# Stansfash/nonstationary-precip

Hardware: NVIDIA B200
Metric: SVGP-Gibbs ELBO steps/s (higher is better)
Workload: dtype f64

## Files before the change

nonstationary_precip_b200/csrc/common.cuh:

```cuda
#pragma once
#include <cuda_runtime.h>
#include <stdint.h>

#define NPGP_OK 0
#define NPGP_EINVAL (-1)
#define NPGP_EUNSUPPORTED (-2)
#define NPGP_EWORKSPACE (-3)

extern "C" long npgp_launch_counter;

#define NPGP_LAUNCH_CHECK()                       \
  do {                                            \
    ++npgp_launch_counter;                        \
    cudaError_t e__ = cudaGetLastError();         \
    if (e__ != cudaSuccess) return (int)e__;      \
  } while (0)

#define NPGP_CUDA(call)                           \
  do {                                            \
    cudaError_t e__ = (call);                     \
    if (e__ != cudaSuccess) return (int)e__;      \
  } while (0)

namespace npgp {

constexpr int kNumSMs = 148;

__device__ __forceinline__ double warp_sum(double v) {
#pragma unroll
  for (int o = 16; o > 0; o >>= 1) v += __shfl_xor_sync(0xffffffffu, v, o);
  return v;
}

__device__ __forceinline__ double block_sum(double v, double* smem ) {
  const int lane = threadIdx.x & 31, w = threadIdx.x >> 5;
  v = warp_sum(v);
  if (lane == 0) smem[w] = v;
  __syncthreads();
  double r = 0.0;
  if (w == 0) {
    r = (lane < (int)((blockDim.x + 31) >> 5)) ? smem[lane] : 0.0;
    r = warp_sum(r);
  }
  __syncthreads();
  return r;
}

__device__ __forceinline__ void st_v2(double* p, double a, double b) {
  *reinterpret_cast<double2*>(p) = make_double2(a, b);
}

static inline int ceil_div(long a, long b) { return (int)((a + b - 1) / b); }

template <int NRC>
struct RowReducer {
  static constexpr int RB = (32 / NRC) > 0 ? (32 / NRC) : 1;
  static constexpr int LINES = RB * NRC;
  static constexpr int PANEL = LINES * 33;
  double* panel;
  int lane;
  __device__ __forceinline__ RowReducer(double* smem_base, int warp, int lane_) : panel(smem_base + warp * PANEL), lane(lane_) {}
  __device__ __forceinline__ void put(int r, int comp, double v) { panel[((r % RB) * NRC + comp) * 33 + lane]  = v; }
  template <class F>
  __device__ __forceinline__ void flush_if_due(int r, int nr, F out) {
    const int slot = r % RB;
    if (slot != RB - 1 && r != nr - 1) return;
    __syncwarp();
    const int nvals = (slot + 1) * NRC;
    for (int v = lane; v < nvals; v += 32) {
      const double* line = panel + v * 33;
      double a0 = 0.0, a1 = 0.0, a2 = 0.0, a3 = 0.0;
#pragma unroll
      for (int k = 0; k < 32; k += 4) {
        a0 += line[k];
        a1 += line[k + 1];
        a2 += line[k + 2];
        a3 += line[k + 3];
      }
      out(r - slot + v / NRC, v % NRC, (a0 + a1) + (a2 + a3));
    }
    __syncwarp();
  }
};

constexpr int kNT = 128;
constexpr int kCPT = 2;
constexpr int kTJ = kNT * kCPT;
constexpr int kTI = 32;

struct GSpec {
  const double* Gm;
  long ldg;
  const double* rowscale;
  const double* rowvec;
  const double* colvec;
};

#ifndef NPGP_GPF_DEPTH
#define NPGP_GPF_DEPTH 4
#endif
template <int CPT, int DEPTH = NPGP_GPF_DEPTH>
struct GPrefetch {
  const double* base;
  long ldg;
  int row_end;
  bool v[CPT], vec;
  double q[DEPTH][CPT];
  __device__ __forceinline__ GPrefetch(const GSpec& g, int jbase, const bool* valid, int vec_ok, int row_begin,
                                       int row_end_)
      : base(g.Gm ? g.Gm + jbase : nullptr), ldg(g.ldg), row_end(row_end_) {
#pragma unroll
    for (int c = 0; c < CPT; ++c) v[c] = valid[c];
    vec = (CPT == 2) && vec_ok && valid[CPT - 1];
#pragma unroll
    for (int k = 0; k < DEPTH; ++k) fetch(row_begin + k, q[k]);
  }
  __device__ __forceinline__ void fetch(int i, double* out) const {
#pragma unroll
    for (int c = 0; c < CPT; ++c) out[c] = 0.0;
    if (base == nullptr || i >= row_end) return;
    const double* grow = base + (long)i * ldg;
    if (vec) {
      const double2 t = *reinterpret_cast<const double2*>(grow);
      out[0] = t.x;
      out[CPT - 1] = t.y;
    } else {
#pragma unroll
      for (int c = 0; c < CPT; ++c)
        if (v[c]) out[c] = grow[c];
    }
  }
  __device__ __forceinline__ void pop(int i, double* out) {
#pragma unroll
    for (int c = 0; c < CPT; ++c) out[c] = q[0][c];
#pragma unroll
    for (int k = 0; k + 1 < DEPTH; ++k)
#pragma unroll
      for (int c = 0; c < CPT; ++c) q[k][c] = q[k + 1][c];
    fetch(i + DEPTH, q[DEPTH - 1]);
  }
};

static inline int pick_rows_per_cta(int n1, int col_tiles, int waves_target) {
  long want = (long)kNumSMs * waves_target;
  long row_ctas = (want + col_tiles - 1) / col_tiles;
  long rpc = (n1 + row_ctas - 1) / row_ctas;
  rpc = ((rpc + kTI - 1) / kTI) * kTI;
  if (rpc < kTI) rpc = kTI;
  return (int)rpc;
}

}
```

nonstationary_precip_b200/csrc/gibbs_full.cu:

```cuda
#include <cstdlib>
#include "common.cuh"
#include "pairmath.cuh"

namespace npgp {


template <int d>
__device__ __forceinline__ void stage_rows_full(int n1, int i0, const double* __restrict__ x1,
                                                const double* __restrict__ S1, double (*sx)[d],
                                                double (*sS)[sym_size(d)], double* sq) {
  constexpr int P = sym_size(d);
  for (int r = threadIdx.x; r < kTI; r += kNT) {
    const int i = i0 + r;
    double S[P];
#pragma unroll
    for (int k = 0; k < d; ++k) sx[r][k] = (i < n1) ? x1[(long)i * d + k] : 0.0;
#pragma unroll
    for (int p = 0; p < P; ++p) S[p] = 0.0;
#pragma unroll
    for (int k = 0; k < d; ++k) S[sym_idx(d, k, k)] = 1.0;
    if (i < n1) {
#pragma unroll
      for (int p = 0; p < P; ++p) S[p] = S1[(long)i * P + p];
    }
#pragma unroll
    for (int p = 0; p < P; ++p) sS[r][p] = S[p];
    sq[r] = sqrt(sqrt(sym_det<d>(S)));
  }
}

template <int d>
__device__ __forceinline__ void load_col_full(int n2, int j, const double* __restrict__ x2,
                                              const double* __restrict__ S2, double* z, double* S, double& q,
                                              bool& valid) {
  constexpr int P = sym_size(d);
  valid = j < n2;
#pragma unroll
  for (int k = 0; k < d; ++k) z[k] = valid ? x2[(long)j * d + k] : 0.0;
#pragma unroll
  for (int p = 0; p < P; ++p) S[p] = 0.0;
#pragma unroll
  for (int k = 0; k < d; ++k) S[sym_idx(d, k, k)] = 1.0;
  if (valid) {
#pragma unroll
    for (int p = 0; p < P; ++p) S[p] = S2[(long)j * P + p];
  }
  q = full_col_factor<d>(sym_det<d>(S));
}

template <int d, bool HAS_U>
__global__ void __launch_bounds__(kNT) gibbs_full_fwd_kernel(int n1, int n2, const double* __restrict__ x1,
                                                             const double* __restrict__ S1,
                                                             const double* __restrict__ x2,
                                                             const double* __restrict__ S2, double jit2,
                                                             const double* __restrict__ scale, double* __restrict__ K,
                                                             long ldk, int vec_ok, const double* __restrict__ u,
                                                             double* __restrict__ Ku, int rows_per_cta) {
  constexpr int P = sym_size(d);
  __shared__ double sx[kTI][d], sS[kTI][P], sq[kTI];
  __shared__ double sexp[256];
  load_exp_table(sexp);
  const int jbase = blockIdx.y * kTJ + threadIdx.x * kCPT;
  const int row_begin = blockIdx.x * rows_per_cta;
  const int row_end = min(n1, row_begin + rows_per_cta);
  const double s = scale ? *scale : 1.0;
  double z[kCPT][d], Sj[kCPT][P], qj[kCPT], uj[kCPT];
  bool valid[kCPT];
#pragma unroll
  for (int c = 0; c < kCPT; ++c) {
    load_col_full<d>(n2, jbase + c, x2, S2, z[c], Sj[c], qj[c], valid[c]);
    qj[c] *= s;
    uj[c] = (HAS_U && valid[c]) ? u[jbase + c] : 0.0;
  }
  for (int i0 = row_begin; i0 < row_end; i0 += kTI) {
    __syncthreads();
    stage_rows_full<d>(n1, i0, x1, S1, sx, sS, sq);
    __syncthreads();
    const int nr = min(kTI, row_end - i0);
#pragma unroll 2
    for (int r = 0; r < nr; ++r) {
      const double k0 = gibbs_full_eval<d>(sx[r], sS[r], sq[r], z[0], Sj[0], qj[0], jit2, sexp);
      const double k1 = gibbs_full_eval<d>(sx[r], sS[r], sq[r], z[1], Sj[1], qj[1], jit2, sexp);
      double* krow = K + (long)(i0 + r) * ldk + jbase;
      if (vec_ok && valid[1]) {
        st_v2(krow, k0, k1);
      } else {
        if (valid[0]) krow[0] = k0;
        if (valid[1]) krow[1] = k1;
      }
      if (HAS_U) {
        double p = warp_sum(fma(k0, uj[0], k1 * uj[1]));
        if ((threadIdx.x & 31) == 0) atomicAdd(&Ku[i0 + r], p);
      }
    }
  }
}


#ifndef NPGP_FULL_BWD_MINB
#define NPGP_FULL_BWD_MINB 2
#endif
template <int d, bool DX1, bool DX2, int CPT>
__global__ void __launch_bounds__(kNT, NPGP_FULL_BWD_MINB) gibbs_full_bwd_kernel(int n1, int n2, const double* __restrict__ x1,
                                                             const double* __restrict__ S1,
                                                             const double* __restrict__ x2,
                                                             const double* __restrict__ S2, double jit2,
                                                             const double* __restrict__ scale, GSpec g, int vec_ok,
                                                             double* __restrict__ d_S1, double* __restrict__ d_x1,
                                                             double* __restrict__ d_S2, double* __restrict__ d_x2,
                                                             double* __restrict__ d_scale, int rows_per_cta) {
  constexpr int P = sym_size(d);
  constexpr int NRC = P + 1 + (DX1 ? d : 0);
  constexpr int NW = kNT / 32;
  __shared__ double sx[kTI][d], sS[kTI][P], sq[kTI], srs[kTI], srv[kTI];
  __shared__ double part[NW][kTI][NRC];
  __shared__ double red[32];
  __shared__ double panels[NW * RowReducer<NRC>::PANEL];
  const int lane = threadIdx.x & 31, warp = threadIdx.x >> 5;
  RowReducer<NRC> rr(panels, warp, lane);
  __shared__ double sexp[256];
  load_exp_table(sexp);
  const int jbase = blockIdx.y * (kNT * CPT) + threadIdx.x * CPT;
  const int row_begin = blockIdx.x * rows_per_cta;
  const int row_end = min(n1, row_begin + rows_per_cta);
  const double s = scale ? *scale : 1.0;
  double z[CPT][d], Sj[CPT][P], qj[CPT], cv[CPT];
  bool valid[CPT];
#pragma unroll
  for (int c = 0; c < CPT; ++c) {
    load_col_full<d>(n2, jbase + c, x2, S2, z[c], Sj[c], qj[c], valid[c]);
    cv[c] = (g.colvec && valid[c]) ? g.colvec[jbase + c] : 0.0;
    qj[c] *= s;
  }
  double cW[CPT][P], cs0[CPT], cxz[CPT][d];
#pragma unroll
  for (int c = 0; c < CPT; ++c) {
    cs0[c] = 0.0;
#pragma unroll
    for (int p = 0; p < P; ++p) cW[c][p] = 0.0;
#pragma unroll
    for (int k = 0; k < d; ++k) cxz[c][k] = 0.0;
  }
  GPrefetch<CPT> gq(g, jbase, valid, vec_ok, row_begin, row_end);

  for (int i0 = row_begin; i0 < row_end; i0 += kTI) {
    __syncthreads();
    stage_rows_full<d>(n1, i0, x1, S1, sx, sS, sq);
    for (int r = threadIdx.x; r < kTI; r += kNT) {
      const int i = i0 + r;
      srs[r] = (g.rowscale && i < n1) ? g.rowscale[i] : 1.0;
      srv[r] = (g.rowvec && i < n1) ? g.rowvec[i] : 0.0;
    }
    __syncthreads();
    const int nr = min(kTI, row_end - i0);
    for (int r = 0; r < nr; ++r) {
      double gv[CPT];
      gq.pop(i0 + r, gv);
#pragma unroll
      for (int c = 0; c < CPT; ++c) gv[c] = fma(srv[r], cv[c], gv[c] * srs[r]);
      double rW[P], rxz[d], rs0 = 0.0;
#pragma unroll
      for (int p = 0; p < P; ++p) rW[p] = 0.0;
#pragma unroll
      for (int k = 0; k < d; ++k) rxz[k] = 0.0;
#pragma unroll
      for (int c = 0; c < CPT; ++c) {
        FullPair<d> pr;
        gibbs_full_eval<d>(sx[r], sS[r], sq[r], z[c], Sj[c], qj[c], jit2, sexp, &pr);
        const double gk = valid[c] ? gv[c] * pr.k : 0.0;
        rs0 += gk;
        cs0[c] += gk;
        const double c2 = -gk * pr.hr2;
        double t[d];
#pragma unroll
        for (int a = 0; a < d; ++a) t[a] = (0.5 * gk) * pr.w[a];
#pragma unroll
        for (int a = 0; a < d; ++a)
#pragma unroll
          for (int b = a; b < d; ++b) {
            const int p = sym_idx(d, a, b);
            const double w = fma(t[a], pr.w[b], c2 * pr.adjA[p]);
            rW[p] += w;
            cW[c][p] += w;
          }
        if (DX1 || DX2) {
#pragma unroll
          for (int k = 0; k < d; ++k) {
            if (DX1) rxz[k] += t[k];
            if (DX2) cxz[c][k] += t[k];
          }
        }
      }
#pragma unroll
      for (int p = 0; p < P; ++p) rr.put(r, p, rW[p]);
      rr.put(r, P, rs0);
      if (DX1) {
#pragma unroll
        for (int k = 0; k < d; ++k) rr.put(r, P + 1 + k, rxz[k]);
      }
      rr.flush_if_due(r, nr, [&](int row, int comp, double v) { part[warp][row][comp] = v; });
    }
    __syncthreads();
    for (int t = threadIdx.x; t < nr * NRC; t += kNT) {
      const int r = t / NRC, comp = t % NRC;
      double v = 0.0;
#pragma unroll
      for (int w = 0; w < NW; ++w) v += part[w][r][comp];
      const int i = i0 + r;
      if (comp < P) {
        atomicAdd(&d_S1[(long)i * P + comp], v);
      } else if (comp == P) {
        double adj[P], det;
        sym_adj_det<d>(sS[r], adj, det);
        const double f = 0.25 * v / det;
#pragma unroll
        for (int p = 0; p < P; ++p) atomicAdd(&d_S1[(long)i * P + p], f * adj[p]);
      } else if (DX1) {
        atomicAdd(&d_x1[(long)i * d + (comp - P - 1)], -4.0 * v);
      }
    }
  }
#pragma unroll
  for (int c = 0; c < CPT; ++c) {
    if (!valid[c]) continue;
    const int j = jbase + c;
    double adj[P], det;
    sym_adj_det<d>(Sj[c], adj, det);
    const double f = 0.25 * cs0[c] / det;
#pragma unroll
    for (int p = 0; p < P; ++p) atomicAdd(&d_S2[(long)j * P + p], fma(f, adj[p], cW[c][p]));
    if (DX2) {
#pragma unroll
      for (int k = 0; k < d; ++k) atomicAdd(&d_x2[(long)j * d + k], 4.0 * cxz[c][k]);
    }
  }
  if (d_scale) {
    double acc_scale = 0.0;
#pragma unroll
    for (int c = 0; c < CPT; ++c) acc_scale += valid[c] ? cs0[c] : 0.0;
    const double t = block_sum(acc_scale / s, red);
    if (threadIdx.x == 0) atomicAdd(d_scale, t);
  }
}

template <int d>
__global__ void sigma_from_h_fwd_kernel(int n, const double* __restrict__ H, const double* __restrict__ Dm,
                                        double* __restrict__ S) {
  constexpr int P = sym_size(d);
  const int i = blockIdx.x * blockDim.x + threadIdx.x;
  if (i >= n) return;
  double h[d], Dl[d * d], out[P];
#pragma unroll
  for (int k = 0; k < d; ++k) h[k] = H[(long)i * d + k];
#pragma unroll
  for (int k = 0; k < d * d; ++k) Dl[k] = Dm[k];
  sigma_from_h_row<d>(h, Dl, out);
#pragma unroll
  for (int p = 0; p < P; ++p) S[(long)i * P + p] = out[p];
}

template <int d>
__global__ void sigma_from_h_bwd_kernel(int n, const double* __restrict__ H, const double* __restrict__ Dm,
                                        const double* __restrict__ dS, double* __restrict__ dH,
                                        double* __restrict__ dDm) {
  constexpr int P = sym_size(d);
  __shared__ double red[32];
  const int i = blockIdx.x * blockDim.x + threadIdx.x;
  double gD[P];
#pragma unroll
  for (int p = 0; p < P; ++p) gD[p] = 0.0;
  if (i < n) {
    double h[d], G[P], gh[d];
#pragma unroll
    for (int k = 0; k < d; ++k) {
      h[k] = H[(long)i * d + k];
      gh[k] = 0.0;
    }
#pragma unroll
    for (int p = 0; p < P; ++p) G[p] = dS[(long)i * P + p];
#pragma unroll
    for (int k = 0; k < d; ++k)
#pragma unroll
      for (int l = 0; l < d; ++l) {
        const int p = (k <= l) ? sym_idx(d, k, l) : sym_idx(d, l, k);
        const double u = h[k] * h[l];
        gh[k] += 4.0 * G[p] * sigmoid20(u * u) * u * h[l];
      }
#pragma unroll
    for (int k = 0; k < d; ++k) dH[(long)i * d + k] += gh[k];
#pragma unroll
    for (int p = 0; p < P; ++p) gD[p] = G[p];
  }
  if (dDm) {
#pragma unroll
    for (int k = 0; k < d; ++k)
#pragma unroll
      for (int l = k; l < d; ++l) {
        const double t = block_sum(gD[sym_idx(d, k, l)], red);
        if (threadIdx.x == 0) {
          atomicAdd(&dDm[k * d + l], 2.0 * Dm[k * d + l] * t);
          if (l != k) atomicAdd(&dDm[l * d + k], 2.0 * Dm[l * d + k] * t);
        }
      }
  }
}


template <int d>
static int launch_full_fwd(int n1, int n2, const double* x1, const double* S1, const double* x2, const double* S2,
                           double jitter, const double* scale, double* K, long ldk, const double* u, double* Ku,
                           cudaStream_t st) {
  const int col_tiles = ceil_div(n2, kTJ);
  const int rpc = pick_rows_per_cta(n1, col_tiles, 16);
  dim3 grid(ceil_div(n1, rpc), col_tiles);
  const int vec_ok = (ldk % 2 == 0) && ((reinterpret_cast<uintptr_t>(K) & 15) == 0);
  if (u)
    gibbs_full_fwd_kernel<d, true><<<grid, kNT, 0, st>>>(n1, n2, x1, S1, x2, S2, 2.0 * jitter, scale, K, ldk, vec_ok, u,
                                                         Ku, rpc);
  else
    gibbs_full_fwd_kernel<d, false><<<grid, kNT, 0, st>>>(n1, n2, x1, S1, x2, S2, 2.0 * jitter, scale, K, ldk, vec_ok,
                                                          u, Ku, rpc);
  NPGP_LAUNCH_CHECK();
  return NPGP_OK;
}

template <int d, int CPT>
static int launch_full_bwd_cpt(int n1, int n2, const double* x1, const double* S1, const double* x2, const double* S2,
                               double jitter, const double* scale, GSpec g, double* d_S1, double* d_x1, double* d_S2,
                               double* d_x2, double* d_scale, cudaStream_t st) {
  const int col_tiles = ceil_div(n2, kNT * CPT);
  const int rpc = pick_rows_per_cta(n1, col_tiles, 8);
  dim3 grid(ceil_div(n1, rpc), col_tiles);
  const int vec_ok = g.Gm ? ((g.ldg % 2 == 0) && ((reinterpret_cast<uintptr_t>(g.Gm) & 15) == 0)) : 0;
#define NPGP_L(A, B)                                                                                               \
  gibbs_full_bwd_kernel<d, A, B, CPT><<<grid, kNT, 0, st>>>(n1, n2, x1, S1, x2, S2, 2.0 * jitter, scale, g, vec_ok, \
                                                            d_S1, d_x1, d_S2, d_x2, d_scale, rpc)
  if (d_x1 && d_x2) NPGP_L(true, true);
  else if (d_x1) NPGP_L(true, false);
  else if (d_x2) NPGP_L(false, true);
  else NPGP_L(false, false);
#undef NPGP_L
  NPGP_LAUNCH_CHECK();
  return NPGP_OK;
}

template <int d>
static int launch_full_bwd(int n1, int n2, const double* x1, const double* S1, const double* x2, const double* S2,
                           double jitter, const double* scale, GSpec g, double* d_S1, double* d_x1, double* d_S2,
                           double* d_x2, double* d_scale, cudaStream_t st) {
  return launch_full_bwd_cpt<d, 2>(n1, n2, x1, S1, x2, S2, jitter, scale, g, d_S1, d_x1, d_S2, d_x2, d_scale, st);
}

}

using namespace npgp;

extern "C" int npgp_gibbs_full_fwd(int d, int n1, int n2, const double* x1, const double* S1, const double* x2,
                                   const double* S2, double jitter, const double* scale, double* K, long ldk,
                                   const double* u, double* Ku, cudaStream_t stream) {
  if (n1 < 0 || n2 < 0 || !K || ldk < n2 || (u && !Ku)) return NPGP_EINVAL;
  if (n1 == 0 || n2 == 0) return NPGP_OK;
  if (!x1 || !S1 || !x2 || !S2) return NPGP_EINVAL;
  if (d == 2) return launch_full_fwd<2>(n1, n2, x1, S1, x2, S2, jitter, scale, K, ldk, u, Ku, stream);
  if (d == 3) return launch_full_fwd<3>(n1, n2, x1, S1, x2, S2, jitter, scale, K, ldk, u, Ku, stream);
  return NPGP_EUNSUPPORTED;
}

extern "C" int npgp_gibbs_full_bwd(int d, int n1, int n2, const double* x1, const double* S1, const double* x2,
                                   const double* S2, double jitter, const double* scale, const double* G, long ldg,
                                   const double* rowscale, const double* rowvec, const double* colvec, double* d_S1,
                                   double* d_x1, double* d_S2, double* d_x2, double* d_scale, cudaStream_t stream) {
  if (n1 < 0 || n2 < 0 || (!G && !rowvec) || (G && ldg < n2) || ((rowvec != nullptr) != (colvec != nullptr)))
    return NPGP_EINVAL;
  if (n1 == 0 || n2 == 0) return NPGP_OK;
  if (!x1 || !S1 || !x2 || !S2 || !d_S1 || !d_S2) return NPGP_EINVAL;
  GSpec g{G, ldg, rowscale, rowvec, colvec};
  if (d == 2) return launch_full_bwd<2>(n1, n2, x1, S1, x2, S2, jitter, scale, g, d_S1, d_x1, d_S2, d_x2, d_scale, stream);
  if (d == 3) return launch_full_bwd<3>(n1, n2, x1, S1, x2, S2, jitter, scale, g, d_S1, d_x1, d_S2, d_x2, d_scale, stream);
  return NPGP_EUNSUPPORTED;
}

extern "C" int npgp_sigma_from_h_fwd(int d, int n, const double* H, const double* Dm, double* S, cudaStream_t stream) {
  if (n < 0 || !Dm) return NPGP_EINVAL;
  if (n == 0) return NPGP_OK;
  if (!H || !S) return NPGP_EINVAL;
  const int nb = ceil_div(n, 256);
  if (d == 2) sigma_from_h_fwd_kernel<2><<<nb, 256, 0, stream>>>(n, H, Dm, S);
  else if (d == 3) sigma_from_h_fwd_kernel<3><<<nb, 256, 0, stream>>>(n, H, Dm, S);
  else return NPGP_EUNSUPPORTED;
  NPGP_LAUNCH_CHECK();
  return NPGP_OK;
}

extern "C" int npgp_sigma_from_h_bwd(int d, int n, const double* H, const double* Dm, const double* dS, double* dH,
                                     double* dDm, cudaStream_t stream) {
  if (n < 0 || !Dm) return NPGP_EINVAL;
  if (n == 0) return NPGP_OK;
  if (!H || !dS || !dH) return NPGP_EINVAL;
  const int nb = ceil_div(n, 256);
  if (d == 2) sigma_from_h_bwd_kernel<2><<<nb, 256, 0, stream>>>(n, H, Dm, dS, dH, dDm);
  else if (d == 3) sigma_from_h_bwd_kernel<3><<<nb, 256, 0, stream>>>(n, H, Dm, dS, dH, dDm);
  else return NPGP_EUNSUPPORTED;
  NPGP_LAUNCH_CHECK();
  return NPGP_OK;
}
```

nonstationary_precip_b200/csrc/pairmath.cuh:

```cuda
#pragma once
#include <math.h>

#include "exp_table.cuh"

#if defined(__CUDACC__)
#define NPGP_HD __host__ __device__ __forceinline__
#else
#define NPGP_HD inline
#endif

namespace npgp {

NPGP_HD double fast_rsqrt(double x) {
#if defined(__CUDA_ARCH__)
  double y;
  asm("rsqrt.approx.ftz.f64 %0, %1;" : "=d"(y) : "d"(x));
  const double h = 0.5 * x;
#pragma unroll
  for (int it = 0; it < 2; ++it) {
    const double e = fma(-h * y, y, 0.5);
    y = fma(y, e, y);
  }
  return y;
#else
  return 1.0 / sqrt(x);
#endif
}

#if defined(__CUDACC__)
__host__ __device__
#endif
NPGP_HD double exp_neg(double x, const double* tab) {
#if defined(__CUDA_ARCH__)
  x = fmax(x, -708.0);
  const double t = fma(x, kInvLn2x256, 6755399441055744.0);
  const int n = __double2loint(t);
  const double nd = t - 6755399441055744.0;
  double r = fma(nd, -kLn2d256Hi, x);
  r = fma(nd, -kLn2d256Lo, r);
  double p = fma(r, 1.0 / 24.0, 1.0 / 6.0);
  p = fma(p, r, 0.5);
  p = fma(p, r, 1.0);
  p = fma(p, r, 1.0);
  const double v = tab[n & 255] * p;
  return __hiloint2double(__double2hiint(v) + ((n >> 8) << 20), __double2loint(v));
#else
  (void)tab;
  return exp(x);
#endif
}

NPGP_HD double fast_rcp(double x) {
#if defined(__CUDA_ARCH__)
  double r;
  asm("rcp.approx.ftz.f64 %0, %1;" : "=d"(r) : "d"(x));
#pragma unroll
  for (int it = 0; it < 2; ++it) {
    const double e = fma(-x, r, 1.0);
    r = fma(r, e, r);
  }
  return r;
#else
  return 1.0 / x;
#endif
}

constexpr int sym_size(int d) { return d * (d + 1) / 2; }

template <int D>
struct DiagPair {
  double k;
  double is[D];
  double dl[D];
};

template <int D>
NPGP_HD double gibbs_diag_eval(const double* xi, const double* ai, double ci, const double* zj, const double* bj,
                               double cj, const double* etab, DiagPair<D>* out = nullptr) {
  double s[D], dl[D], pre[D + 1], suf[D + 1];
#pragma unroll
  for (int d = 0; d < D; ++d) {
    s[d] = ai[d] + bj[d];
    dl[d] = xi[d] - zj[d];
  }
  pre[0] = 1.0;
#pragma unroll
  for (int d = 0; d < D; ++d) pre[d + 1] = pre[d] * s[d];
  suf[D] = 1.0;
#pragma unroll
  for (int d = D - 1; d >= 0; --d) suf[d] = suf[d + 1] * s[d];
  const double P = pre[D];
  double num = 0.0;
  double pe[D];
#pragma unroll
  for (int d = 0; d < D; ++d) {
    pe[d] = pre[d] * suf[d + 1];
    num = fma(dl[d] * dl[d], pe[d], num);
  }
  const double r = fast_rsqrt(P);
  const double r2 = r * r;
  const double k = (ci * cj) * r * exp_neg(-num * r2, etab);
  if (out) {
    out->k = k;
#pragma unroll
    for (int d = 0; d < D; ++d) {
      out->is[d] = pe[d] * r2;
      out->dl[d] = dl[d];
    }
  }
  return k;
}

template <int d>
NPGP_HD void sym_adj_det(const double* m, double* adj, double& det);

template <>
NPGP_HD void sym_adj_det<2>(const double* m, double* adj, double& det) {
  adj[0] = m[2];
  adj[1] = -m[1];
  adj[2] = m[0];
  det = fma(m[0], m[2], -m[1] * m[1]);
}

template <>
NPGP_HD void sym_adj_det<3>(const double* m, double* adj, double& det) {
  adj[0] = fma(m[3], m[5], -m[4] * m[4]);
  adj[1] = fma(m[2], m[4], -m[1] * m[5]);
  adj[2] = fma(m[1], m[4], -m[2] * m[3]);
  adj[3] = fma(m[0], m[5], -m[2] * m[2]);
  adj[4] = fma(m[1], m[2], -m[0] * m[4]);
  adj[5] = fma(m[0], m[3], -m[1] * m[1]);
  det = fma(m[0], adj[0], fma(m[1], adj[1], m[2] * adj[2]));
}

template <int d>
NPGP_HD double sym_det(const double* m) {
  double adj[sym_size(d)], det;
  sym_adj_det<d>(m, adj, det);
  return det;
}

template <int d>
NPGP_HD void sym_matvec(const double* m, const double* v, double* y);
template <>
NPGP_HD void sym_matvec<2>(const double* m, const double* v, double* y) {
  y[0] = fma(m[0], v[0], m[1] * v[1]);
  y[1] = fma(m[1], v[0], m[2] * v[1]);
}
template <>
NPGP_HD void sym_matvec<3>(const double* m, const double* v, double* y) {
  y[0] = fma(m[0], v[0], fma(m[1], v[1], m[2] * v[2]));
  y[1] = fma(m[1], v[0], fma(m[3], v[1], m[4] * v[2]));
  y[2] = fma(m[2], v[0], fma(m[4], v[1], m[5] * v[2]));
}

NPGP_HD int sym_idx(int d, int k, int l) {
  return k * d - (k * (k - 1)) / 2 + (l - k);
}

template <int d>
NPGP_HD void sym_adj_det_shifted(const double* At, const double* adjA, double lam, double* adjB, double& detB);
template <>
NPGP_HD void sym_adj_det_shifted<2>(const double* At, const double* adjA, double lam, double* adjB, double& detB) {
  (void)adjA;
  const double b0 = At[0] + lam, b2 = At[2] + lam;
  adjB[0] = b2;
  adjB[1] = -At[1];
  adjB[2] = b0;
  detB = fma(b0, b2, -At[1] * At[1]);
}
template <>
NPGP_HD void sym_adj_det_shifted<3>(const double* At, const double* adjA, double lam, double* adjB, double& detB) {
  const double b0 = At[0] + lam, b3 = At[3] + lam, b5 = At[5] + lam;
  adjB[0] = fma(b3, b5, -At[4] * At[4]);
  adjB[1] = fma(-lam, At[1], adjA[1]);
  adjB[2] = fma(-lam, At[2], adjA[2]);
  adjB[3] = fma(b0, b5, -At[2] * At[2]);
  adjB[4] = fma(-lam, At[4], adjA[4]);
  adjB[5] = fma(b0, b3, -At[1] * At[1]);
  detB = fma(b0, adjB[0], fma(At[1], adjB[1], At[2] * adjB[2]));
}

template <int d>
struct FullPair {
  double k;
  double w[d];
  double adjA[sym_size(d)];
  double hr2;
};

template <int d>
NPGP_HD double full_col_factor(double det_Sj) {
  return ((d == 2) ? 2.0 : 2.8284271247461900976) * sqrt(sqrt(det_Sj));
}

template <int d>
NPGP_HD double gibbs_full_eval(const double* xi, const double* Si, double qi, const double* zj, const double* Sj,
                               double qj, double jit2, const double* etab, FullPair<d>* out = nullptr) {
  constexpr int P = sym_size(d);
  double At[P], adjA[P], adjB[P], detA, detB, dl[d], v[d];
#pragma unroll
  for (int p = 0; p < P; ++p) At[p] = Si[p] + Sj[p];
#pragma unroll
  for (int k = 0; k < d; ++k) dl[k] = xi[k] - zj[k];
  sym_adj_det<d>(At, adjA, detA);
  sym_adj_det_shifted<d>(At, adjA, jit2, adjB, detB);
  sym_matvec<d>(adjB, dl, v);
  double dv = 0.0;
#pragma unroll
  for (int k = 0; k < d; ++k) dv = fma(dl[k], v[k], dv);
  const double nidetB2 = -2.0 * fast_rcp(detB);
  const double r = fast_rsqrt(detA);
  const double k = (qi * qj) * r * exp_neg(dv * nidetB2, etab);
  if (out) {
    out->k = k;
    out->hr2 = 0.5 * r * r;
#pragma unroll
    for (int a = 0; a < d; ++a) out->w[a] = -v[a] * nidetB2;
#pragma unroll
    for (int p = 0; p < P; ++p) out->adjA[p] = adjA[p];
  }
  return k;
}

NPGP_HD double softplus20(double t) { return t > 20.0 ? t : log1p(exp(t)); }
NPGP_HD double sigmoid20(double t) { return t > 20.0 ? 1.0 : 1.0 / (1.0 + exp(-t)); }

template <int d>
NPGP_HD void sigma_from_h_row(const double* h, const double* Dm , double* S ) {
#pragma unroll
  for (int k = 0; k < d; ++k)
#pragma unroll
    for (int l = k; l < d; ++l) {
      const double u = h[k] * h[l];
      S[sym_idx(d, k, l)] = softplus20(u * u) + Dm[k * d + l] * Dm[k * d + l];
    }
}

}
```

Measured before the change: 234.5.

## Restructure Gibbs full backward kernel: packed row records, folded scales, higher occupancy

Rewrites the full-covariance Gibbs backward kernel so that per-row data (x, S, q times rowscale, q times rowvec) sit in one aligned shared-memory record read with double2 loads. Column data are packed with the half-scale and colvec folded in, which reduces per-pair multiplies and register footprint. The launch-bounds minimum-blocks hint is raised to 3 and the prefetch depth cut to 3 to allow more resident CTAs. The per-row atomic epilogue is reorganised so each thread handles a whole row and fuses the determinant-gradient term into a single atomic per component. Column S is re-read from global memory at the end instead of being held in registers. The tighter register cap risks spills in f64 code.

Result: faster. 238.9 (median of 6 runs) (+1.9%).

```diff
diff --git a/nonstationary_precip_b200/csrc/common.cuh b/nonstationary_precip_b200/csrc/common.cuh
--- a/nonstationary_precip_b200/csrc/common.cuh
+++ b/nonstationary_precip_b200/csrc/common.cuh
@@ -69,9 +69,9 @@
     const int nvals = (slot + 1) * NRC;
     for (int v = lane; v < nvals; v += 32) {
       const double* line = panel + v * 33;
-      double a0 = 0.0, a1 = 0.0, a2 = 0.0, a3 = 0.0;
+      double a0 = line[0], a1 = line[1], a2 = line[2], a3 = line[3];
 #pragma unroll
-      for (int k = 0; k < 32; k += 4) {
+      for (int k = 4; k < 32; k += 4) {
         a0 += line[k];
         a1 += line[k + 1];
         a2 += line[k + 2];
diff --git a/nonstationary_precip_b200/csrc/gibbs_full.cu b/nonstationary_precip_b200/csrc/gibbs_full.cu
--- a/nonstationary_precip_b200/csrc/gibbs_full.cu
+++ b/nonstationary_precip_b200/csrc/gibbs_full.cu
@@ -97,11 +97,8 @@
 }
 
 
-#ifndef NPGP_FULL_BWD_MINB
-#define NPGP_FULL_BWD_MINB 2
-#endif
 template <int d, bool DX1, bool DX2, int CPT>
-__global__ void __launch_bounds__(kNT, NPGP_FULL_BWD_MINB) gibbs_full_bwd_kernel(int n1, int n2, const double* __restrict__ x1,
+__global__ void __launch_bounds__(kNT, 3) gibbs_full_bwd_kernel(int n1, int n2, const double* __restrict__ x1,
                                                              const double* __restrict__ S1,
                                                              const double* __restrict__ x2,
                                                              const double* __restrict__ S2, double jit2,
@@ -112,7 +109,9 @@
   constexpr int P = sym_size(d);
   constexpr int NRC = P + 1 + (DX1 ? d : 0);
   constexpr int NW = kNT / 32;
-  __shared__ double sx[kTI][d], sS[kTI][P], sq[kTI], srs[kTI], srv[kTI];
+  constexpr int NF = d + P + 2;
+  constexpr int RREC = (d + P + 2 + 1) & ~1;
+  __shared__ __align__(16) double srow[kTI][RREC];
   __shared__ double part[NW][kTI][NRC];
   __shared__ double red[32];
   __shared__ double panels[NW * RowReducer<NRC>::PANEL];
@@ -124,13 +123,20 @@
   const int row_begin = blockIdx.x * rows_per_cta;
   const int row_end = min(n1, row_begin + rows_per_cta);
   const double s = scale ? *scale : 1.0;
-  double z[CPT][d], Sj[CPT][P], qj[CPT], cv[CPT];
+  double cc[CPT][NF];
   bool valid[CPT];
 #pragma unroll
   for (int c = 0; c < CPT; ++c) {
-    load_col_full<d>(n2, jbase + c, x2, S2, z[c], Sj[c], qj[c], valid[c]);
-    cv[c] = (g.colvec && valid[c]) ? g.colvec[jbase + c] : 0.0;
-    qj[c] *= s;
+    double z[d], Sj[P], qj;
+    load_col_full<d>(n2, jbase + c, x2, S2, z, Sj, qj, valid[c]);
+    const double qh = 0.5 * s * qj;
+    const double cv = (g.colvec && valid[c]) ? g.colvec[jbase + c] : 0.0;
+#pragma unroll
+    for (int k = 0; k < d; ++k) cc[c][k] = z[k];
+#pragma unroll
+    for (int p = 0; p < P; ++p) cc[c][d + p] = Sj[p];
+    cc[c][d + P] = qh;
+    cc[c][d + P + 1] = qh * cv;
   }
   double cW[CPT][P], cs0[CPT], cxz[CPT][d];
 #pragma unroll
@@ -141,54 +147,67 @@
 #pragma unroll
     for (int k = 0; k < d; ++k) cxz[c][k] = 0.0;
   }
-  GPrefetch<CPT> gq(g, jbase, valid, vec_ok, row_begin, row_end);
+  GPrefetch<CPT, 3> gq(g, jbase, valid, vec_ok, row_begin, row_end);
 
   for (int i0 = row_begin; i0 < row_end; i0 += kTI) {
     __syncthreads();
-    stage_rows_full<d>(n1, i0, x1, S1, sx, sS, sq);
     for (int r = threadIdx.x; r < kTI; r += kNT) {
       const int i = i0 + r;
-      srs[r] = (g.rowscale && i < n1) ? g.rowscale[i] : 1.0;
-      srv[r] = (g.rowvec && i < n1) ? g.rowvec[i] : 0.0;
+      double* rec = srow[r];
+      double S[P];
+#pragma unroll
+      for (int p = 0; p < P; ++p) S[p] = 0.0;
+#pragma unroll
+      for (int k = 0; k < d; ++k) S[sym_idx(d, k, k)] = 1.0;
+      if (i < n1) {
+#pragma unroll
+        for (int p = 0; p < P; ++p) S[p] = S1[(long)i * P + p];
+      }
+#pragma unroll
+      for (int k = 0; k < d; ++k) rec[k] = (i < n1) ? x1[(long)i * d + k] : 0.0;
+#pragma unroll
+      for (int p = 0; p < P; ++p) rec[d + p] = S[p];
+      const double qi = sqrt(sqrt(sym_det<d>(S)));
+      rec[d + P] = (g.rowscale && i < n1) ? qi * g.rowscale[i] : qi;
+      rec[d + P + 1] = (g.rowvec && i < n1) ? qi * g.rowvec[i] : 0.0;
     }
     __syncthreads();
     const int nr = min(kTI, row_end - i0);
     for (int r = 0; r < nr; ++r) {
       double gv[CPT];
       gq.pop(i0 + r, gv);
-#pragma unroll
-      for (int c = 0; c < CPT; ++c) gv[c] = fma(srv[r], cv[c], gv[c] * srs[r]);
-      double rW[P], rxz[d], rs0 = 0.0;
-#pragma unroll
-      for (int p = 0; p < P; ++p) rW[p] = 0.0;
-#pragma unroll
-      for (int k = 0; k < d; ++k) rxz[k] = 0.0;
+      double ri[RREC];
+#pragma unroll
+      for (int k = 0; k < RREC; k += 2) {
+        const double2 t = *reinterpret_cast<const double2*>(&srow[r][k]);
+        ri[k] = t.x;
+        ri[k + 1] = t.y;
+      }
+      double rW[P], rxz[d], rs0;
 #pragma unroll
       for (int c = 0; c < CPT; ++c) {
         FullPair<d> pr;
-        gibbs_full_eval<d>(sx[r], sS[r], sq[r], z[c], Sj[c], qj[c], jit2, sexp, &pr);
-        const double gk = valid[c] ? gv[c] * pr.k : 0.0;
-        rs0 += gk;
-        cs0[c] += gk;
-        const double c2 = -gk * pr.hr2;
+        gibbs_full_pair<d>(ri, ri + d, cc[c], cc[c] + d, jit2, sexp, pr);
+        const double hgk = pr.e * fma(ri[d + P] * gv[c], cc[c][d + P], ri[d + P + 1] * cc[c][d + P + 1]);
+        cs0[c] += hgk;
+        const double c2 = -hgk * pr.r2;
         double t[d];
 #pragma unroll
-        for (int a = 0; a < d; ++a) t[a] = (0.5 * gk) * pr.w[a];
+        for (int a = 0; a < d; ++a) t[a] = hgk * pr.w[a];
 #pragma unroll
         for (int a = 0; a < d; ++a)
 #pragma unroll
           for (int b = a; b < d; ++b) {
             const int p = sym_idx(d, a, b);
             const double w = fma(t[a], pr.w[b], c2 * pr.adjA[p]);
-            rW[p] += w;
+            rW[p] = c ? rW[p] + w : w;
             cW[c][p] += w;
           }
-        if (DX1 || DX2) {
-#pragma unroll
-          for (int k = 0; k < d; ++k) {
-            if (DX1) rxz[k] += t[k];
-            if (DX2) cxz[c][k] += t[k];
-          }
+        rs0 = c ? rs0 + hgk : hgk;
+#pragma unroll
+        for (int k = 0; k < d; ++k) {
+          if (DX1) rxz[k] = c ? rxz[k] + t[k] : t[k];
+          if (DX2) cxz[c][k] += t[k];
         }
       }
 #pragma unroll
@@ -201,22 +220,23 @@
       rr.flush_if_due(r, nr, [&](int row, int comp, double v) { part[warp][row][comp] = v; });
     }
     __syncthreads();
-    for (int t = threadIdx.x; t < nr * NRC; t += kNT) {
-      const int r = t / NRC, comp = t % NRC;
-      double v = 0.0;
-#pragma unroll
-      for (int w = 0; w < NW; ++w) v += part[w][r][comp];
-      const int i = i0 + r;
-      if (comp < P) {
-        atomicAdd(&d_S1[(long)i * P + comp], v);
-      } else if (comp == P) {
-        double adj[P], det;
-        sym_adj_det<d>(sS[r], adj, det);
-        const double f = 0.25 * v / det;
-#pragma unroll
-        for (int p = 0; p < P; ++p) atomicAdd(&d_S1[(long)i * P + p], f * adj[p]);
-      } else if (DX1) {
-        atomicAdd(&d_x1[(long)i * d + (comp - P - 1)], -4.0 * v);
+    for (int r = threadIdx.x; r < nr; r += kNT) {
+      double v[NRC];
+#pragma unroll
+      for (int comp = 0; comp < NRC; ++comp) {
+        v[comp] = part[0][r][comp];
+#pragma unroll
+        for (int w = 1; w < NW; ++w) v[comp] += part[w][r][comp];
+      }
+      const long i = i0 + r;
+      double adj[P], det;
+      sym_adj_det<d>(&srow[r][d], adj, det);
+      const double f = 0.5 * v[P] / det;
+#pragma unroll
+      for (int p = 0; p < P; ++p) atomicAdd(&d_S1[i * P + p], fma(f, adj[p], v[p]));
+      if (DX1) {
+#pragma unroll
+        for (int k = 0; k < d; ++k) atomicAdd(&d_x1[i * d + k], -4.0 * v[P + 1 + k]);
       }
     }
   }
@@ -225,8 +245,8 @@
     if (!valid[c]) continue;
     const int j = jbase + c;
     double adj[P], det;
-    sym_adj_det<d>(Sj[c], adj, det);
-    const double f = 0.25 * cs0[c] / det;
+    sym_adj_det<d>(S2 + (long)j * P, adj, det);
+    const double f = 0.5 * cs0[c] / det;
 #pragma unroll
     for (int p = 0; p < P; ++p) atomicAdd(&d_S2[(long)j * P + p], fma(f, adj[p], cW[c][p]));
     if (DX2) {
@@ -238,7 +258,7 @@
     double acc_scale = 0.0;
 #pragma unroll
     for (int c = 0; c < CPT; ++c) acc_scale += valid[c] ? cs0[c] : 0.0;
-    const double t = block_sum(acc_scale / s, red);
+    const double t = block_sum(2.0 * acc_scale / s, red);
     if (threadIdx.x == 0) atomicAdd(d_scale, t);
   }
 }
diff --git a/nonstationary_precip_b200/csrc/pairmath.cuh b/nonstationary_precip_b200/csrc/pairmath.cuh
--- a/nonstationary_precip_b200/csrc/pairmath.cuh
+++ b/nonstationary_precip_b200/csrc/pairmath.cuh
@@ -182,21 +182,13 @@
 }
 
 template <int d>
-struct FullPair {
-  double k;
-  double w[d];
-  double adjA[sym_size(d)];
-  double hr2;
-};
-
-template <int d>
 NPGP_HD double full_col_factor(double det_Sj) {
   return ((d == 2) ? 2.0 : 2.8284271247461900976) * sqrt(sqrt(det_Sj));
 }
 
 template <int d>
 NPGP_HD double gibbs_full_eval(const double* xi, const double* Si, double qi, const double* zj, const double* Sj,
-                               double qj, double jit2, const double* etab, FullPair<d>* out = nullptr) {
+                               double qj, double jit2, const double* etab) {
   constexpr int P = sym_size(d);
   double At[P], adjA[P], adjB[P], detA, detB, dl[d], v[d];
 #pragma unroll
@@ -211,16 +203,38 @@
   for (int k = 0; k < d; ++k) dv = fma(dl[k], v[k], dv);
   const double nidetB2 = -2.0 * fast_rcp(detB);
   const double r = fast_rsqrt(detA);
-  const double k = (qi * qj) * r * exp_neg(dv * nidetB2, etab);
-  if (out) {
-    out->k = k;
-    out->hr2 = 0.5 * r * r;
-#pragma unroll
-    for (int a = 0; a < d; ++a) out->w[a] = -v[a] * nidetB2;
-#pragma unroll
-    for (int p = 0; p < P; ++p) out->adjA[p] = adjA[p];
-  }
-  return k;
+  return (qi * qj) * r * exp_neg(dv * nidetB2, etab);
+}
+
+template <int d>
+struct FullPair {
+  double e;
+  double w[d];
+  double adjA[sym_size(d)];
+  double r2;
+};
+
+template <int d>
+NPGP_HD void gibbs_full_pair(const double* xi, const double* Si, const double* zj, const double* Sj, double jit2,
+                             const double* etab, FullPair<d>& out) {
+  constexpr int P = sym_size(d);
+  double At[P], adjB[P], detA, detB, dl[d], v[d];
+#pragma unroll
+  for (int p = 0; p < P; ++p) At[p] = Si[p] + Sj[p];
+#pragma unroll
+  for (int k = 0; k < d; ++k) dl[k] = xi[k] - zj[k];
+  sym_adj_det<d>(At, out.adjA, detA);
+  sym_adj_det_shifted<d>(At, out.adjA, jit2, adjB, detB);
+  sym_matvec<d>(adjB, dl, v);
+  const double idetB2 = 2.0 * fast_rcp(detB);
+#pragma unroll
+  for (int a = 0; a < d; ++a) out.w[a] = v[a] * idetB2;
+  double q = dl[0] * out.w[0];
+#pragma unroll
+  for (int k = 1; k < d; ++k) q = fma(dl[k], out.w[k], q);
+  const double r = fast_rsqrt(detA);
+  out.e = r * exp_neg(-q, etab);
+  out.r2 = r * r;
 }
 
 NPGP_HD double softplus20(double t) { return t > 20.0 ? t : log1p(exp(t)); }
```
